# wakensky/parameter_server

Measured on AMD Instinct MI355X. Metric: aggregated kv-pairs/s (device-resident), N-way sparse push merge at 1/2/4/8 GPU, higher is better.
Workload: dtype f32; 1 GPU; cfg2: 8 pushes x 131072 sorted unique uint64 keys + f32 values, 10% shared keys (U=956,827); 64 such (channel,time) aggregates per GPU per step; global_batch=64, input_layout=arena, parallelism=key-range shards evenDivide(1); worker-sliced ingress, no data-path collective

## Files before the change

### include/psg.h

```cpp
#ifndef PSG_H_
#define PSG_H_

#include <stddef.h>
#include <stdint.h>

#ifdef __cplusplus
extern "C" {
#endif

#define PSG_ABI_VERSION 1
#define PSG_MAX_VALUE_ARRAYS 4

typedef enum psg_status {
  PSG_OK = 0,
  PSG_ERR_ARG = -1,
  PSG_ERR_UNMATCHED = -2,
  PSG_ERR_RANGE = -3,
  PSG_ERR_NO_TIME = -4,
  PSG_ERR_OOM = -5,
  PSG_ERR_DEVICE = -6,
  PSG_ERR_UNSORTED = -7,
  PSG_ERR_SIZE = -8,
  PSG_ERR_CHANNEL = -9,
  PSG_ERR_EMPTY_KEYS = -10,
// ... 77 lines not shown

int psg_plan_create(int device, int dtype, int m, unsigned flags,
                    const psg_merge_job* jobs, int njobs, psg_plan** out);
int psg_plan_max_push(void);
int psg_plan_run(psg_plan* plan, void* stream);
int psg_plan_run_stage(psg_plan* plan, int stage, void* stream);
int psg_plan_matched(psg_plan* plan, uint64_t* matched);
#define PSG_KERNEL_TILE 0
#define PSG_KERNEL_TILE64 1
#define PSG_KERNEL_PACKED 2
#define PSG_KERNEL_DENSE 3
#define PSG_KERNEL_CURSOR 4
#define PSG_KERNEL_PACKED_CURSOR 5
int psg_plan_form(psg_plan* plan, int* form);
int psg_plan_bytes(psg_plan* plan, uint64_t* bytes, uint64_t* kv_pairs);
int psg_plan_destroy(psg_plan* plan);

int psg_gather_dev(int dtype, const uint64_t* dkeys, uint64_t nd,
                   const void* dvals, const uint64_t* req, uint64_t nreq,
                   void* out, unsigned long long* matched, void* stream);

int psg_key_union_dev(const uint64_t* a, uint64_t na, const uint64_t* b,
                      uint64_t nb, uint64_t* out, uint64_t* nout,
                      void* stream);

typedef struct psg_nway psg_nway;
int psg_nway_max_push(void);
int psg_nway_create(int device, int dtype, int m, unsigned flags, int npush,
                    const uint64_t* const* keys, const uint64_t* n, const void* const* vals,
                    uint64_t* out_keys, void* const* out_vals, psg_nway** out);
// ... 188 lines not shown
```

### parameter_server_amd/_lib.py

```python
from __future__ import annotations

import ctypes as C
import os

_HERE = os.path.dirname(os.path.abspath(__file__))
LIB_PATH = os.environ.get("PSG_LIB_PATH") or os.path.join(_HERE, "libpsg.so")

PSG_OK = 0
PSG_ERR_ARG = -1
PSG_ERR_UNMATCHED = -2
PSG_ERR_RANGE = -3
PSG_ERR_NO_TIME = -4
PSG_ERR_OOM = -5
PSG_ERR_DEVICE = -6
PSG_ERR_UNSORTED = -7
PSG_ERR_SIZE = -8
PSG_ERR_CHANNEL = -9
PSG_ERR_EMPTY_KEYS = -10
PSG_ERR_SIGNATURE = -11
PSG_KC_SIG = 1
PSG_KC_KEYS = 2
PSG_KC_ERASE = 4
PSG_MAX_SIG_LEN = 2048

# ... 81 lines not shown
    "psg_key_cache_clear": (C.c_int, [_p, C.c_int]),
    "psg_push_compressed": (C.c_int, [_p, C.c_int, C.c_int, _u64, _u64, _p, _sz, C.c_int,
                                      _p, _p]),
    "psg_key_cache_bytes": (C.c_int, [_p, C.c_int, _psz]),
    "psg_received_shape": (C.c_int, [_p, C.c_int, C.POINTER(C.c_int), _psz, _psz]),
    "psg_received": (C.c_int, [_p, C.c_int, C.c_int, C.POINTER(_p)]),
    "psg_gather": (C.c_int, [_p, C.c_int, _p, _sz, _p, _psz]),
    "psg_plan_create": (C.c_int, [C.c_int, C.c_int, C.c_int, C.c_uint,
                                  C.POINTER(MergeJob), C.c_int, C.POINTER(_p)]),
    "psg_plan_max_push": (C.c_int, []),
    "psg_plan_run": (C.c_int, [_p, _p]),
    "psg_plan_run_stage": (C.c_int, [_p, C.c_int, _p]),
    "psg_plan_matched": (C.c_int, [_p, _pu64]),
    "psg_plan_bytes": (C.c_int, [_p, _pu64, _pu64]),
    "psg_plan_form": (C.c_int, [_p, C.POINTER(C.c_int)]),
    "psg_plan_destroy": (C.c_int, [_p]),
    "psg_gather_dev": (C.c_int, [C.c_int, _p, _u64, _p, _p, _u64, _p, _p, _p]),
    "psg_key_union_dev": (C.c_int, [_p, _u64, _p, _u64, _p, _pu64, _p]),
    "psg_shard_bounds": (C.c_int, [_sz, _pu64]),
    "psg_slice_dev": (C.c_int, [_p, _u64, _u64, _u64, _p, C.c_int, _p, _p]),
    "psg_crc32c_dev": (C.c_int, [_p, _p, _u64, _u64, _p, _p, _p]),
    "psg_snappy_uncompress_dev": (C.c_int, [_p, _p, _u64, _p, _p, _p, _p]),
    "psg_snappy_uncompressed_length": (C.c_int, [_p, _sz, _psz]),
    "psg_freq_resize": (C.c_int, [_p, C.c_int, C.c_int, C.c_int]),
    "psg_freq_clear": (C.c_int, [_p, C.c_int]),
    "psg_freq_empty": (C.c_int, [_p, C.c_int, C.POINTER(C.c_int)]),
    "psg_freq_insert": (C.c_int, [_p, C.c_int, _p, _p, _sz]),
    "psg_freq_query": (C.c_int, [_p, C.c_int, _p, _sz, C.c_int, _p, _psz]),
    "psg_freq_insert_dev": (C.c_int, [_p, C.c_int, _p, _p, _sz, _p]),
    "psg_freq_query_scratch_bytes": (_sz, [_sz]),
# ... 125 lines not shown
```

### parameter_server_amd/csrc/psg_device.h

```cpp
#pragma once
#include <hip/hip_runtime.h>
#include <stdint.h>

namespace psg {
namespace dev {

__device__ __forceinline__ uint64_t wave_search(const uint64_t* __restrict__ S,
                                                uint64_t n, uint64_t key,
                                                bool upper, int lane) {
  uint64_t lo = 0, hi = n;
  while (hi > lo) {
    const uint64_t len = hi - lo;
    const uint64_t step = (len + 63) >> 6;
    const uint64_t idx = lo + (uint64_t)(lane + 1) * step - 1;
    bool pred = true;
    if (idx < hi) {
      const uint64_t s = S[idx];
      pred = upper ? (s > key) : (s >= key);
    }
    const unsigned long long mask = __ballot(pred);
    if (mask == 0) {
      lo = hi;
      break;
    }
// ... 93 lines not shown
      if (lane >= d) s += y;
    }
    if (lane < kW) wsum[lane] = s;
  }
  __syncthreads();
  *total = wsum[kW - 1];
  return (w > 0 ? wsum[w - 1] : 0u) + x - v;
}

__device__ __forceinline__ uint32_t bucket_scale(uint64_t r32, uint32_t nb) {
  const float f = (float)nb * 4294967296.0f * (1.0f - 0x1p-20f) *
                  __builtin_amdgcn_rcpf((float)(r32 + 1ull));
  return f >= 4294967295.0f ? 0xffffffffu : (uint32_t)f;
}

template <typename V>
__device__ __forceinline__ V fold_step(V acc, int lp, int p, V v,
                                       bool parallel, bool cont) {
  if (p == 0 && !cont) return v;
  if (!parallel) {
    const bool gap = (lp >= 0) ? (p - lp > 1) : (cont && p > 0);
    if (gap) acc = acc + V(0);
  }
  return acc + v;
}


}
}
```

### parameter_server_amd/csrc/psg_internal.h

```cpp
#pragma once

#include <hip/hip_runtime.h>
#include <stdint.h>

namespace psg {

constexpr int kMaxPush = 4096;
constexpr int kMaxM = 4;
constexpr int kTileSlots = 1024;
#ifndef PSG_PACK_TS
#define PSG_PACK_TS 2048
#endif
constexpr int kPackTileSlots = PSG_PACK_TS;
constexpr int kWideSlots = 2048;

constexpr uint32_t kFlagParallel = 1u;
constexpr uint32_t kFlagCont = 2u;
constexpr uint32_t kFlagLastTile = 4u;

enum PartMode : uint32_t { kSearch = 0, kStream = 1 };
constexpr uint32_t kStreamChunk = 512;

struct JobDev {
  const uint64_t* dkeys;
// ... 53 lines not shown
struct DenseCheck {
  const uint64_t* keys;
  uint64_t n;
  const uint64_t* D;
  uint64_t nd;
  unsigned long long* out;
};

hipError_t launch_partition(const JobDev* d_jobs, const uint32_t* d_split_item_job,
                            uint32_t nsplit_items, const uint64_t* d_items,
                            uint32_t nitems, hipStream_t stream, bool xcd = false);
hipError_t launch_aggregate_tile(int dtype, int m, const TileDesc* d_tiles, uint32_t ntiles,
                                 int form, hipStream_t stream);
uint32_t bucket_index_words(uint32_t tile_slots);
hipError_t launch_bucket_index(const TileDesc* d_tiles, uint32_t ntiles, uint32_t tile_slots,
                               uint32_t* out,
                               hipStream_t stream);
constexpr int kPackCursorPushes = 256;
hipError_t launch_aggregate_tile_packed(int dtype, int m, const TileDesc* d_tiles,
                                        uint32_t ntiles, hipStream_t stream,
                                        const CursorChunk* d_chunks = nullptr,
                                        uint32_t nchunks = 0, uint32_t* bx = nullptr);
hipError_t launch_aggregate_dense(int dtype, int m, const TileDesc* d_tiles, uint32_t ntiles,
                                  hipStream_t stream);
hipError_t launch_dense_check(const DenseCheck* checks, uint32_t nchecks, const uint64_t* items,
                              uint64_t nitems, hipStream_t stream);
hipError_t launch_gather(int dtype, const uint64_t* dkeys, uint64_t nd,
                         const void* dvals, const uint64_t* req, uint64_t nreq,
                         void* out, unsigned long long* matched,
                         hipStream_t stream);
struct HostCopyDesc {
// ... 116 lines not shown
```

### parameter_server_amd/csrc/psg_runtime.hip

```cpp
#include <hip/hip_runtime.h>
#include <chrono>

#include <algorithm>
#include <cmath>
#include <iterator>
#include <cstdarg>
#include <cstdio>
#include <cstdlib>
#include <cstring>
#include <deque>
#include <map>
#include <memory>
#include <mutex>
#include <string>
#include <unordered_map>
#include <vector>

#include "../../include/psg.h"
#include "psg_host.h"
#include "psg_internal.h"

using psg::JobDev;

namespace {
// ... 120 lines not shown
  std::vector<JobDev> h;
  struct JobInfo {
    uint32_t np = 0, ntiles = 0;
    std::vector<uint64_t> pn;
    std::vector<uint32_t> slot;
    uint32_t ncaller = 0;
    uint32_t* seg = nullptr;
    uint32_t segq = 1;
    unsigned long long* fail = nullptr;
    uint32_t kr = 0;
    uint32_t nch = 0;
  };
  std::vector<JobInfo> info;
  uint32_t ntiles = 0, nitems = 0, nsplit = 0;
  bool split_once = false;
  bool all_search = false;
  void* blob = nullptr;
  size_t blob_bytes = 0;
  JobDev* d_jobs = nullptr;
  psg::TileDesc* d_tiles = nullptr;
  uint32_t* d_split_items = nullptr;
  uint64_t* d_items = nullptr;
  char* himg[2] = {nullptr, nullptr};
  const void* himg_dev[2] = {nullptr, nullptr};
  bool zero_copy = true;
  size_t himg_cap[2] = {0, 0};
  hipEvent_t himg_ev[2] = {nullptr, nullptr};
  int himg_cur = 0;

  std::vector<uint64_t> last_shape;
// ... 138 lines not shown
      for (JobInfo& I : info) {
        I.nch = (uint32_t)((I.ntiles + per - 1) / per);
        nc += I.nch;
      }
      nchunks = (uint32_t)nc;
    } else {
      nchunks = 0;
    }
    size_t off = align_up(sizeof(JobDev) * jobs.size(), 256);
    const size_t tiles_off = off;
    off = align_up(off + sizeof(psg::TileDesc) * tiles, 256);
    const bool use_index = index && !dense;
    const uint32_t iw = psg::bucket_index_words(tile);
    const size_t index_off = off;
    if (use_index) off = align_up(off + 4 * (size_t)iw * tiles, 256);
    const size_t sitems_off = off;
    off = align_up(off + 4 * sitems, 256);
    const size_t items_off = off;
    off = align_up(off + 8 * items, 256);
    const size_t cjobs_off = off;
    if (cursor) off = align_up(off + sizeof(psg::CursorJob) * jobs.size(), 256);
    const size_t chunks_off = off;
    if (cursor || pcursor) off = align_up(off + sizeof(psg::CursorChunk) * nchunks, 256);
    const size_t zero_off = off;
    size_t fail_cur = zero_off;
    {
      uint64_t npall = 0;
      for (const JobInfo& I : info) npall += I.np;
      off = align_up(off + 8 * npall, 256);
    }
// ... 45 lines not shown
    if (himg_ev[ib]) HIP_TRY(hipEventSynchronize(himg_ev[ib]));
    else HIP_TRY(hipEventCreateWithFlags(&himg_ev[ib], hipEventDisableTiming));
    if (off > himg_cap[ib]) {
      if (himg[ib]) HIP_TRY(hipHostFree(himg[ib]));
      himg[ib] = nullptr;
      himg_cap[ib] = 0;
      HIP_TRY(hipHostMalloc((void**)&himg[ib], off));
      himg_cap[ib] = off;
      himg_dev[ib] = nullptr;
      void* dp = nullptr;
      if (hipHostGetDevicePointer(&dp, himg[ib], 0) == hipSuccess) himg_dev[ib] = dp;
      else (void)hipGetLastError();
    }
    char* img = himg[ib];
    memset(img + zero_off, 0, zero_end - zero_off);
    psg::TileDesc* htiles = (psg::TileDesc*)(img + tiles_off);
    uint32_t* hsitems = (uint32_t*)(img + sitems_off);
    uint64_t* hitems = (uint64_t*)(img + items_off);
    uint64_t tcur = 0, icur = 0, scur = 0;
    for (size_t j = 0; j < jobs.size(); ++j) {
      const JobSpec& s = jobs[j];
      JobInfo& I = info[j];
      const Offs& o = offs[j];
      const uint32_t np = I.np, nt = I.ntiles;
      uint64_t* hk = (uint64_t*)(img + o.pk);
      uint64_t* hv = (uint64_t*)(img + o.pv);
      for (uint32_t p = 0; p < np; ++p) {
        const uint32_t c = I.slot[p];
        hk[p] = (uint64_t)s.pkeys[c];
        for (int i = 0; i < m; ++i) hv[(size_t)p * m + i] = (uint64_t)s.pvals[(size_t)c * m + i];
// ... 147 lines not shown
      cb.d[1] = psg::HostCopyDesc{(const char*)himg_dev[ib] + zero_off, base + zero_off,
                                  (uint64_t)(off - zero_off)};
      HIP_TRY(psg::launch_host_copy_batch(cb, strm));
    } else if (same) {
      HIP_TRY(hipMemcpyAsync(blob, img, tiles_off, hipMemcpyHostToDevice, strm));
      HIP_TRY(hipMemcpyAsync(base + zero_off, img + zero_off, off - zero_off,
                             hipMemcpyHostToDevice, strm));
    } else if (zc_ok) {
      HIP_TRY(psg::launch_host_copy(blob, himg_dev[ib], off, strm));
    } else {
      HIP_TRY(hipMemcpyAsync(blob, img, off, hipMemcpyHostToDevice, strm));
    }
    if (cacheable) last_shape.swap(shape);
    else last_shape.clear();
    HIP_TRY(hipEventRecord(himg_ev[ib], strm));
    if (use_index)
      HIP_TRY(psg::launch_bucket_index(d_tiles, ntiles, tile,
                                       (uint32_t*)((char*)blob + index_off), strm));
    split_once = index && nsplit > 0 && !dense && !cursor && !pcursor;
    all_search = true;
    for (const JobDev& d : h) all_search = all_search && d.mode == psg::kSearch;
    if (split_once)
      HIP_TRY(psg::launch_partition(d_jobs, d_split_items, nsplit, nullptr, 0, strm));
    if (!async) HIP_TRY(hipStreamSynchronize(strm));
    return PSG_OK;
  }

  int run_stage(int stage, hipStream_t s) const {
    if (h.empty()) return PSG_OK;
    if (stage == 0) {
      if (cursor || pcursor)
        HIP_TRY(hipMemsetAsync(d_zero, 0, zero_bytes, s));
      else if (!dense)
        HIP_TRY(psg::launch_partition(d_jobs, d_split_items, split_once ? 0u : nsplit, d_items,
                                      nitems, s, all_search));
    } else if (cursor)
      HIP_TRY(psg::launch_aggregate_cursor(dtype, m, (int)ckr, d_cjobs, d_chunks, nchunks, d_bx, s));
    else if (dense)
      HIP_TRY(psg::launch_aggregate_dense(dtype, m, d_tiles, ntiles, s));
// ... 783 lines not shown
  return PSG_OK;
}

int psg_plan_form(psg_plan* plan, int* form) {
  if (!plan || !form) return fail(PSG_ERR_ARG, "null argument");
  const JobTable& T = plan->table;
  *form = T.cursor ? PSG_KERNEL_CURSOR
          : T.pcursor ? PSG_KERNEL_PACKED_CURSOR
          : T.dense ? PSG_KERNEL_DENSE
          : T.pack  ? PSG_KERNEL_PACKED
          : T.wide  ? PSG_KERNEL_TILE64
                    : PSG_KERNEL_TILE;
  return PSG_OK;
}

int psg_plan_bytes(psg_plan* plan, uint64_t* bytes, uint64_t* kv) {
  if (!plan) return fail(PSG_ERR_ARG, "null plan");
  if (bytes) *bytes = plan->bytes;
  if (kv) *kv = plan->kv;
  return PSG_OK;
}

int psg_plan_destroy(psg_plan* plan) {
  if (!plan) return PSG_OK;
  (void)hipSetDevice(plan->table.device);
  plan->table.release();
  delete plan;
  return PSG_OK;
}

// ... 1415 lines not shown
```

### parameter_server_amd/csrc/psg_tile.hip

```cpp
#include <hip/hip_runtime.h>
#include <stdint.h>

#include "psg_device.h"
#include "psg_internal.h"

#define AS1 __attribute__((address_space(1)))
#ifndef KCAP64
#define KCAP64 7
#endif

namespace psg {

#ifndef PSG_SKELETON
#define PSG_SKELETON 0
#endif
#ifdef PSG_PHASES
constexpr int kPhTiles = 1 << 17;
__device__ uint32_t g_phase[kPhTiles][8];
#define PH(i) do { const unsigned long long _t = clock64(); \
    ph_acc[i] += (uint32_t)(_t - ph_t); ph_t = _t; } while (0)
#else
#define PH(i) do { } while (0)
#endif

// ... 144 lines not shown
                                 __HIP_MEMORY_SCOPE_AGENT);
        const uint32_t len = b > a ? (b - a < (uint32_t)kTS ? b - a : (uint32_t)kTS) : 0u;
        pln[lane] = len;
        pkp[lane] = (uint64_t)(kp + a);
#pragma unroll
        for (int mi = 0; mi < M; ++mi) pvp[lane * M + mi] = (uint64_t)(vp[mi] + a);
        nr = (len + 63u) >> 6;
      }
      const uint32_t x = wave_scan_incl(nr);
      if (lane < kGroup) rpre[lane + 1] = x;
      if (lane == 0) rpre[0] = 0;
    }
  };
  const uint32_t s0 = 4u * (uint32_t)tid;
  const uint32_t* Bg = T.bt;
  const bool dma = PSG_DDMA && nt == (uint32_t)kTS && ((uintptr_t)Dg & 15u) == 0u &&
                   ((uintptr_t)Bg & 15u) == 0u;
  auto issue_dma = [&]() {
#pragma unroll
    for (int j = 0; j < 2; ++j) {
      const uint32_t c = 2u * w + (uint32_t)j;
      dma16(Dg + 128u * c + 2u * (uint32_t)lane, (char*)dk + 1024u * c);
    }
    static_assert(kNB / 512 <= kNW, "one 1-KB unit of the bucket table per wave at most");
    if (Bg && w < (uint32_t)kNB / 512u)
      dma16((const char*)Bg + 1024u * w + 16u * (uint32_t)lane, (char*)bt32 + 1024u * w);
  };
  if (dma && w != 0) issue_dma();
  if (np) load_tables(0);
  if (dma && w == 0) issue_dma();
  if (!dma) {
    uint64_t d[4];
    if (s0 + 3u < nt && ((uintptr_t)Dg & 15u) == 0u) {
      const u64x2 x0 = __builtin_nontemporal_load((const AS1 u64x2*)(Dg + s0));
      const u64x2 x1 = __builtin_nontemporal_load((const AS1 u64x2*)(Dg + s0 + 2));
      d[0] = x0.x; d[1] = x0.y; d[2] = x1.x; d[3] = x1.y;
    } else {
#pragma unroll
      for (int j = 0; j < 4; ++j) d[j] = s0 + j < nt ? G(Dg)[s0 + j] : ~0ull;
    }
    u32x2 btw = {0u, 0u};
    if (Bg) btw = __builtin_nontemporal_load((const AS1 u32x2*)Bg + tid);
#pragma unroll
    for (int j = 0; j < 4; ++j) dk[s0 + j] = d[j];
    if (Bg) {
      bt32[tid * (kBPT / 2)] = btw.x;
      bt32[tid * (kBPT / 2) + 1] = btw.y;
    }
    __builtin_amdgcn_s_waitcnt(0x0f70);
  }
  if (cont) {
    V a0[M][4];
#pragma unroll
    for (int mi = 0; mi < M; ++mi)
#pragma unroll
      for (int j = 0; j < 4; ++j)
        a0[mi][j] = s0 + j < nt ? G((const V*)T.out[mi] + T.slot0)[s0 + j] : V(0);
    __builtin_amdgcn_s_waitcnt(0x0f70);
    if constexpr (kFuse) {
      *(u32x4*)&cnt32[8 * tid] = u32x4{__float_as_uint(a0[0][0]), 0u, __float_as_uint(a0[0][1]), 0u};
      *(u32x4*)&cnt32[8 * tid + 4] = u32x4{__float_as_uint(a0[0][2]), 0u, __float_as_uint(a0[0][3]), 0u};
    } else {
#pragma unroll
// ... 6 lines not shown
    *(u32x4*)&cnt32[8 * tid + 4] = u32x4{0u, 0u, 0u, 0u};
  } else {
#pragma unroll
    for (int mi = 0; mi < M; ++mi)
#pragma unroll
      for (int j = 0; j < 4; ++j) acc[mi][s0 + j] = V(0);
  }
  if constexpr (kFuse) {
  } else if constexpr (kCntW) {
    *(u32x4*)&cnt32[4 * tid] = u32x4{0u, 0u, 0u, 0u};
  } else {
    cnt32[2 * tid] = 0u;
    cnt32[2 * tid + 1] = 0u;
  }
  if (tid < 4) dk[kTS + tid] = ~0ull;
  if (Bg) {
    if (tid == 0) bt[kNB] = (uint16_t)nt;
  } else {
    uint32_t z = 0;
#pragma unroll
    for (int i = 0; i < kBPT / 2; ++i) bt32[tid * (kBPT / 2) + i] = z;
  }
  if (tid == 0) pcarry = -1;
  if (dma)
    lds_barrier();
  else
    __syncthreads();
  PH(0);

  uint32_t done = 0, U = np ? uni(rpre[np < (uint32_t)kGroup ? np : kGroup]) : 0u;
  uint32_t g0 = 0;
  uint32_t nrw = 0, ua = 0, Rw = 0;
  uint32_t re[kCap];
// ... 55 lines not shown
  const uint64_t klo = uni64(dk[0]);
  const uint64_t khi = uni64(dk[nt - 1]);
  const uint64_t range = khi - klo;
  const int bits = range ? 64 - __builtin_clzll(range) : 0;
  const int s2 = bits > 32 ? bits - 32 : 0;
  const uint64_t r32 = range >> s2;
  const uint32_t mul = dev::bucket_scale(r32, kNB);
  auto bucket = [&](uint64_t k) -> uint32_t {
    const uint64_t x = (k - klo) >> s2;
    const uint32_t xs = x > r32 ? 0xffffffffu : (uint32_t)x;
    const uint32_t b = __umulhi(xs, mul);
    return b < (uint32_t)(kNB - 1) ? b : (uint32_t)(kNB - 1);
  };


  if (!Bg) {
  const u64x2 y0 = *(const u64x2*)&dk[s0];
  const u64x2 y1 = *(const u64x2*)&dk[s0 + 2];
  const uint64_t dd[4] = {y0.x, y0.y, y1.x, y1.y};
#pragma unroll
  for (int j = 0; j < 4; ++j)
    if (s0 + j < nt)
    {
      const uint32_t b = bucket(dd[j]);
      __hip_atomic_fetch_add(&bt32[b >> 1], 1u << (16 * (b & 1u)), __ATOMIC_RELAXED,
                             __HIP_MEMORY_SCOPE_WORKGROUP);
    }
  __syncthreads();
  {
    uint32_t e[kBPT];
#pragma unroll
// ... 226 lines not shown
    } else {
#pragma unroll
      for (int j = 0; j < 4; ++j)
        if (s0 + j < nt) GW(o)[j] = res[mi][j];
    }
  }
  PH(6);
#ifdef PSG_PHASES
  if (tid == 0 && ti < (uint32_t)kPhTiles)
    for (int i = 0; i < 8; ++i) g_phase[ti][i] = ph_acc[i];
#endif
}

template <int kTSl>
__global__ __launch_bounds__(kTSl / 4) void bucket_index_kernel(
    const TileDesc* __restrict__ tiles, uint32_t ntiles, uint32_t* __restrict__ out) {
  constexpr int kNT = kTSl / 4;
  constexpr int kNW = kNT / 64;
  constexpr int kNB = kTSl;
  constexpr int kBPT = kNB / kNT;
  __shared__ __attribute__((aligned(16))) uint32_t bt32[(kNB + 8) / 2];
  __shared__ uint32_t wsum[kNW];
  const uint32_t ti = blockIdx.x;
  if (ti >= ntiles) return;
  const TileDesc& T = tiles[ti];
  const uint32_t nt = T.nt;
  const uint64_t* Dg = T.dk;
  const int tid = threadIdx.x, lane = tid & 63;
  const uint32_t w = uni((uint32_t)tid >> 6);
  const uint32_t s0 = 4u * (uint32_t)tid;
  const uint64_t klo = G(Dg)[0];
  const uint64_t khi = G(Dg)[nt - 1];
  const uint64_t range = khi - klo;
  const int bits = range ? 64 - __builtin_clzll(range) : 0;
  const int s2 = bits > 32 ? bits - 32 : 0;
  const uint64_t r32 = range >> s2;
  const uint32_t mul = dev::bucket_scale(r32, kNB);
#pragma unroll
  for (int i = 0; i < kBPT / 2; ++i) bt32[tid * (kBPT / 2) + i] = 0u;
  __syncthreads();
#pragma unroll
  for (int j = 0; j < 4; ++j)
    if (s0 + j < nt) {
      const uint64_t x = (G(Dg)[s0 + j] - klo) >> s2;
      const uint32_t b = x > r32 ? (uint32_t)(kNB - 1) : __umulhi((uint32_t)x, mul);
      __hip_atomic_fetch_add(&bt32[b >> 1], 1u << (16 * (b & 1u)), __ATOMIC_RELAXED,
                             __HIP_MEMORY_SCOPE_WORKGROUP);
    }
  __syncthreads();
  uint32_t e[kBPT];
#pragma unroll
  for (int i = 0; i < kBPT / 2; ++i) {
    const uint32_t h = bt32[tid * (kBPT / 2) + i];
    e[2 * i] = h & 0xffffu;
    e[2 * i + 1] = h >> 16;
  }
  uint32_t tot = 0;
#pragma unroll
  for (int j = 0; j < kBPT; ++j) {
    const uint32_t c = e[j];
    e[j] = tot;
    tot += c;
  }
  const uint32_t x = wave_scan_incl(tot);
  if (lane == 63) wsum[w] = x;
  __syncthreads();
  uint32_t off = x - tot;
#pragma unroll
  for (uint32_t v = 0; v < (uint32_t)kNW - 1u; ++v) off += v < w ? wsum[v] : 0u;
  uint32_t* o = out + (size_t)ti * (kNB / 2);
#pragma unroll
  for (int i = 0; i < kBPT / 2; ++i)
    o[tid * (kBPT / 2) + i] = (e[2 * i] + off) | (e[2 * i + 1] + off) << 16;
}

#ifndef PSG_PAD_LDS
#define PSG_PAD_LDS 0
#endif
template <typename V, int M>
hipError_t go(const TileDesc* t, uint32_t n, int form, hipStream_t s) {
  if (form == 1)
    hipLaunchKernelGGL((tile_kernel<V, M, 64>), dim3(n), dim3(nt_of(64)), PSG_PAD_LDS, s, t, n);
  else
    hipLaunchKernelGGL((tile_kernel<V, M, 32>), dim3(n), dim3(nt_of(32)), PSG_PAD_LDS, s, t, n);
  return hipGetLastError();
}

template <typename V>
// ... 4 lines not shown
    case 3: return go<V, 3>(t, n, form, s);
    case 4: return go<V, 4>(t, n, form, s);
    default: return hipErrorInvalidValue;
  }
}

}

#ifdef PSG_PHASES
extern "C" int psg_debug_phases(uint32_t* out, uint32_t ntiles) {
  if (ntiles > (uint32_t)kPhTiles) ntiles = kPhTiles;
  return hipMemcpyFromSymbol(out, HIP_SYMBOL(g_phase), (size_t)ntiles * 32) == hipSuccess ? 0 : -1;
}
#endif

uint32_t bucket_index_words(uint32_t tile_slots) { return tile_slots / 2u; }

hipError_t launch_bucket_index(const TileDesc* d_tiles, uint32_t ntiles, uint32_t tile_slots,
                               uint32_t* out, hipStream_t stream) {
  if (ntiles == 0) return hipSuccess;
  switch (tile_slots) {
    case 1024:
      hipLaunchKernelGGL(bucket_index_kernel<1024>, dim3(ntiles), dim3(256), 0, stream, d_tiles,
                         ntiles, out);
      break;
    case 2048:
      hipLaunchKernelGGL(bucket_index_kernel<2048>, dim3(ntiles), dim3(512), 0, stream, d_tiles,
                         ntiles, out);
      break;
    case 4096:
      hipLaunchKernelGGL(bucket_index_kernel<4096>, dim3(ntiles), dim3(1024), 0, stream, d_tiles,
                         ntiles, out);
      break;
    default:
      return hipErrorInvalidValue;
  }
  return hipGetLastError();
}

hipError_t launch_aggregate_tile(int dtype, int m, const TileDesc* d_tiles, uint32_t ntiles,
                                 int form, hipStream_t stream) {
  if (ntiles == 0) return hipSuccess;
  return dtype == 0 ? launch_m<float>(m, d_tiles, ntiles, form, stream)
                    : launch_m<double>(m, d_tiles, ntiles, form, stream);
}

}
// ... 1 lines not shown
```

### parameter_server_amd/csrc/psg_tile_cursor.hip

```cpp
#include <hip/hip_runtime.h>
#include <stdint.h>

#include "psg_device.h"
#include "psg_internal.h"

#define AS1 __attribute__((address_space(1)))

namespace psg {

namespace {

template <typename T>
__device__ __forceinline__ const AS1 T* G(const T* p) {
  return (const AS1 T*)p;
}
template <typename T>
__device__ __forceinline__ AS1 T* GW(T* p) {
  return (AS1 T*)p;
}

constexpr int kTS = kTileSlots;
constexpr int kNT = kTS / 4;
constexpr int kNW = kNT / 64;
constexpr int kNB = kTS;
// ... 157 lines not shown
      }
      if (g0 == 0) {
        uint64_t d[4];
        if (s0 + 3u < nt && ((uintptr_t)Dg & 15u) == 0u) {
          const u64x2 x0 = __builtin_nontemporal_load((const AS1 u64x2*)(Dg + s0));
          const u64x2 x1 = __builtin_nontemporal_load((const AS1 u64x2*)(Dg + s0 + 2));
          d[0] = x0.x; d[1] = x0.y; d[2] = x1.x; d[3] = x1.y;
        } else {
#pragma unroll
          for (int j = 0; j < 4; ++j) {
            uint64_t o = ~0ull;
            asm volatile("" : "+v"(o));
            d[j] = s0 + j < nt ? G(Dg)[s0 + j] : o;
          }
        }
        const u32x2 btw =
            __builtin_nontemporal_load((const AS1 u32x2*)(J.bt + (size_t)t * (kNB / 2)) + tid);
        V a0[M][4];
#pragma unroll
        for (int mi = 0; mi < M; ++mi)
#pragma unroll
          for (int j = 0; j < 4; ++j)
            a0[mi][j] = (cont && s0 + j < nt) ? G((const V*)J.out[mi] + slot0)[s0 + j] : V(0);
#pragma unroll
        for (int j = 0; j < 4; ++j) {
          dk[s0 + j] = d[j];
#pragma unroll
          for (int mi = 0; mi < M; ++mi) acc[mi][s0 + j] = a0[mi][j];
        }
        {
          uint32_t z = 0, o = ~0u;
          asm volatile("" : "+v"(z), "+v"(o));
          *(u32x4*)&cnt[s0] = u32x4{z, z, z, z};
          if (tid < 4) dk[kTS + tid] = (uint64_t)o << 32 | o;
        }
        *(u32x2*)&bt32[2 * tid] = btw;
        if (tid == 0) bt[kNB] = (uint16_t)nt;
        __syncthreads();
      }

      uint32_t inp = 0;
      uint32_t ends[kPPW];
      uint32_t ovf = 0;
#pragma unroll
      for (int p = 0; p < kPPW; ++p) {
        ends[p] = qc[p];
        bool closed = qn[p] >= np;
#pragma unroll
        for (int r = 0; r < kRR; ++r) {
          const int rr = p * kRR + r;
          if ((uint32_t)r < kr && !closed) {
            const bool in = ((hv >> rr) & 1u) && (open || ek[rr] < nxt);
            const uint64_t out = __ballot(!in);
// ... 228 lines not shown
```

### parameter_server_amd/csrc/psg_tile_packed.hip

```cpp
#include <hip/hip_runtime.h>
#include <stdint.h>

#include "psg_device.h"
#include "psg_internal.h"

#define AS1 __attribute__((address_space(1)))

namespace psg {

namespace {

template <typename T>
__device__ __forceinline__ const AS1 T* G(const T* p) {
  return (const AS1 T*)p;
}
template <typename T>
__device__ __forceinline__ AS1 T* GW(T* p) {
  return (AS1 T*)p;
}

#ifndef PSG_SKELETON
#define PSG_SKELETON 0
#endif

// ... 330 lines not shown
      emax = y > emax ? y : emax;
    }
    if (in) {
      pre[ql + 1] = X;
#pragma nounroll
      for (uint32_t e = X - lv; e < X; ++e) ep[e] = (uint8_t)ql;
    }
    if (lane_id() == 0u) {
      __hip_atomic_fetch_add(&gsh[0], fit, __ATOMIC_RELAXED, __HIP_MEMORY_SCOPE_WORKGROUP);
      __hip_atomic_fetch_max(&gsh[1], emax, __ATOMIC_RELAXED, __HIP_MEMORY_SCOPE_WORKGROUP);
    }
    if (t == 0u) pre[0] = 0;
  };
  const uint32_t s0i = 4u * (uint32_t)tid;
  const uint32_t* Bg = T.bt;
  const bool dma = !CUR && PSG_DDMA && nt == (uint32_t)kTS && ((uintptr_t)Dg & 15u) == 0u &&
                   ((uintptr_t)Bg & 15u) == 0u;
  auto issue_dma = [&]() {
#pragma unroll
    for (int j = 0; j < 2; ++j) {
      const uint32_t c = 2u * w + (uint32_t)j;
      dma16(Dg + 128u * c + 2u * (uint32_t)lane, (char*)dk + 1024u * c);
    }
    static_assert(kNB / 512 <= kNW, "one 1-KB unit of the bucket table per wave at most");
    if (Bg && w < (uint32_t)kNB / 512u)
      dma16((const char*)Bg + 1024u * w + 16u * (uint32_t)lane, (char*)bt32 + 1024u * w);
  };
  if (dma && w >= 2) issue_dma();
  if (np) {
    if constexpr (!CUR) tables_a(0);
  }
  if (dma && w < 2) issue_dma();
  if (!dma) {
    uint64_t d[4];
    if (s0i + 3u < nt && ((uintptr_t)Dg & 15u) == 0u) {
      const u64x2 x0 = *(const AS1 u64x2*)(Dg + s0i);
      const u64x2 x1 = *(const AS1 u64x2*)(Dg + s0i + 2);
      d[0] = x0.x; d[1] = x0.y; d[2] = x1.x; d[3] = x1.y;
    } else {
#pragma unroll
      for (int j = 0; j < 4; ++j) d[j] = s0i + j < nt ? G(Dg)[s0i + j] : ~0ull;
    }
    u32x2 btw = {0u, 0u};
    if (Bg) btw = __builtin_nontemporal_load((const AS1 u32x2*)Bg + tid);
#pragma unroll
    for (int j = 0; j < 4; ++j) dk[s0i + j] = d[j];
    if (Bg) *(u32x2*)&bt[tid * kBPT] = btw;
    __builtin_amdgcn_s_waitcnt(0x0f70);
  }
  uint32_t cx = 0, clv = 0;
  if constexpr (CUR) {
    if (np) clv = cur_a(0, true, &cx);
  }

  uint32_t ones = ~0u, one = 1u;
  if constexpr (CUR) asm volatile("" : "+v"(ones), "+v"(one));
  if (cont) {
    V a0[M][4];
#pragma unroll
    for (int mi = 0; mi < M; ++mi)
#pragma unroll
      for (int j = 0; j < 4; ++j)
// ... 4 lines not shown
#pragma unroll
      for (int j = 0; j < 4; ++j) acc[mi][s0i + j] = a0[mi][j];
  } else {
#pragma unroll
    for (int mi = 0; mi < M; ++mi)
#pragma unroll
      for (int j = 0; j < 4; ++j) acc[mi][s0i + j] = V(0);
  }
#pragma unroll
  for (int j = 0; j < 4; ++j) lastl[s0i + j] = (uint16_t)one;
  if (tid < 8) dk[kTS + tid] = (uint64_t)ones << 32 | ones;
  {
    uint32_t z = 0;
    asm volatile("" : "+v"(z));
    if (!Bg) *(u32x2*)&bt[tid * kBPT] = u32x2{z, z};
    if (Bg && tid == 0) bt[kNB] = (uint16_t)nt;
  }
  if (tid == 0) pcarry = (int)ones;
  if (dma)
    lds_barrier();
  else
    __syncthreads();
  if (np) {
    if constexpr (CUR) cur_b(0, clv, cx);
    else tables_b(0);
  }
  if (dma)
    lds_barrier();
  else
    __syncthreads();

// ... 92 lines not shown
        e[j] = tot;
        tot += c;
      }
      const uint32_t x = wave_scan_incl(tot);
      if (lane_id() == 63u) wsum[w] = x;
      __syncthreads();
      uint32_t off = x - tot;
#pragma unroll
      for (uint32_t v = 0; v < (uint32_t)kNW - 1u; ++v) off += v < w ? wsum[v] : 0u;
      const u32x2 o = {(e[0] + off) | (e[1] + off) << 16, (e[2] + off) | (e[3] + off) << 16};
      *(u32x2*)&bt[t * kBPT] = o;
      if (t == 0) bt[kNB] = (uint16_t)nt;
    }
    __syncthreads();
  };
  if (!Bg) build_bt(false);

  for (;;) {
    if (!U) {
      g0 += gp;
      if (g0 >= np) break;
#pragma unroll
      for (int j = 0; j < 4; ++j) lastl[s0i + j] = lastl[s0i + j] == gp + 1u ? 1 : 0;
      if constexpr (CUR) {
        uint32_t x;
        const uint32_t lv = cur_a(g0, false, &x);
        __syncthreads();
        cur_b(g0, lv, x);
      } else {
        tables_a(g0);
        __syncthreads();
// ... 167 lines not shown
                  if (j < lane && s == sl) lowest = false;
                }
                if (lowest) {
                  apply();
                  pend = false;
                }
              }
            }
          }
        }
        if (w == wl && lane == 63) pcarry = mylast;
      }
      __syncthreads();
    }
    if (done + kNW * Rw < U || g0 + gp < np) {
      if (Bg) {
        const uint32_t t = 64u * w + lane_id();
        *(u32x2*)&bt[t * kBPT] = __builtin_nontemporal_load((const AS1 u32x2*)Bg + t);
        __syncthreads();
      } else {
        build_bt(true);
      }
    }

    done += kNW * Rw;
    if (done < U) {
      load_pass();
      continue;
    }
    U = 0;
    if (w == 0 && lane_id() == 0u) pcarry = -1;
  }

// ... 96 lines not shown
```

### parameter_server_amd/kv_vector.py

```python
from __future__ import annotations

import ctypes as C
from dataclasses import dataclass, field
from typing import List, Optional, Sequence

import numpy as np

from . import _lib
from ._lib import PSG_F32, PSG_F64, PSG_PARALLEL_MATCH, PSG_SERIAL_MATCH

KEY_ALL = (0, (1 << 64) - 1)


def _np_dtype(dtype: int):
    return np.float32 if dtype == PSG_F32 else np.float64


def _ptr(a: np.ndarray) -> int:
    return a.ctypes.data


@dataclass
class Message:

# ... 165 lines not shown
            cj[j].push_n = C.cast(pn, C.POINTER(C.c_uint64))
            cj[j].out = C.cast(out, C.POINTER(C.c_void_p))
        h = C.c_void_p()
        flags = (flags & ~PSG_PARALLEL_MATCH) | (PSG_PARALLEL_MATCH if parallel_match
                                                 else PSG_SERIAL_MATCH)
        _lib.check(self._L.psg_plan_create(device, dtype, m, flags, cj, len(jobs),
                                           C.byref(h)))
        self._h = h
        self.npush_total = sum(len(J["push_keys"]) for J in jobs)
        b, kv = C.c_uint64(), C.c_uint64()
        _lib.check(self._L.psg_plan_bytes(h, C.byref(b), C.byref(kv)))
        self.bytes, self.kv_pairs = b.value, kv.value
        f = C.c_int()
        _lib.check(self._L.psg_plan_form(h, C.byref(f)))
        self.form = f.value

    def run(self, stream: Optional[int] = None) -> None:
        _lib.check(self._L.psg_plan_run(self._h, stream or None))

    def run_stage(self, stage: int, stream: Optional[int] = None) -> None:
        _lib.check(self._L.psg_plan_run_stage(self._h, stage, stream or None))

    def matched(self) -> np.ndarray:
        out = np.zeros(max(1, self.npush_total), np.uint64)
        _lib.check(self._L.psg_plan_matched(
            self._h, out.ctypes.data_as(C.POINTER(C.c_uint64))))
        return out[: self.npush_total]

    def close(self):
        if getattr(self, "_h", None):
# ... 103 lines not shown
```

Measured before the change: 182.6 billion kv-pairs/s.

## Compress bucket index to 4-bit counts decoded in-kernel with wave scan

```diff
diff --git a/include/psg.h b/include/psg.h
--- a/include/psg.h
+++ b/include/psg.h
@@ -115,6 +115,7 @@
 #define PSG_KERNEL_PACKED_CURSOR 5
 int psg_plan_form(psg_plan* plan, int* form);
 int psg_plan_bytes(psg_plan* plan, uint64_t* bytes, uint64_t* kv_pairs);
+int psg_plan_index_info(psg_plan* plan, uint64_t* index_bytes, uint64_t* marked_tiles);
 int psg_plan_destroy(psg_plan* plan);
 
 int psg_gather_dev(int dtype, const uint64_t* dkeys, uint64_t nd,
diff --git a/parameter_server_amd/_lib.py b/parameter_server_amd/_lib.py
--- a/parameter_server_amd/_lib.py
+++ b/parameter_server_amd/_lib.py
@@ -119,6 +119,7 @@
     "psg_plan_matched": (C.c_int, [_p, _pu64]),
     "psg_plan_bytes": (C.c_int, [_p, _pu64, _pu64]),
     "psg_plan_form": (C.c_int, [_p, C.POINTER(C.c_int)]),
+    "psg_plan_index_info": (C.c_int, [_p, _pu64, _pu64]),
     "psg_plan_destroy": (C.c_int, [_p]),
     "psg_gather_dev": (C.c_int, [C.c_int, _p, _u64, _p, _p, _u64, _p, _p, _p]),
     "psg_key_union_dev": (C.c_int, [_p, _u64, _p, _u64, _p, _pu64, _p]),
diff --git a/parameter_server_amd/csrc/psg_device.h b/parameter_server_amd/csrc/psg_device.h
--- a/parameter_server_amd/csrc/psg_device.h
+++ b/parameter_server_amd/csrc/psg_device.h
@@ -131,6 +131,78 @@
   return f >= 4294967295.0f ? 0xffffffffu : (uint32_t)f;
 }
 
+template <int kNB>
+struct BucketIndexWords {
+  static_assert(kNB == 1024 || kNB == 2048 || kNB == 4096, "8, 16 or 32 B per lane");
+  uint32_t x[kNB / 512];
+};
+
+template <int kNB>
+__device__ __forceinline__ BucketIndexWords<kNB> bucket_index_load(const uint32_t* ix, int lane) {
+  typedef uint32_t v2 __attribute__((ext_vector_type(2)));
+  typedef uint32_t v4 __attribute__((ext_vector_type(4)));
+  BucketIndexWords<kNB> r;
+  if constexpr (kNB == 1024) {
+    const v2 a = __builtin_nontemporal_load(
+        (const __attribute__((address_space(1))) v2*)ix + lane);
+    r.x[0] = a.x; r.x[1] = a.y;
+  } else {
+#pragma unroll
+    for (int i = 0; i < kNB / 2048; ++i) {
+      const v4 a = __builtin_nontemporal_load(
+          (const __attribute__((address_space(1))) v4*)ix + lane * (kNB / 2048) + i);
+      r.x[4 * i] = a.x; r.x[4 * i + 1] = a.y; r.x[4 * i + 2] = a.z; r.x[4 * i + 3] = a.w;
+    }
+  }
+  return r;
+}
+
+__device__ __forceinline__ uint32_t wave_scan_incl_dpp(uint32_t x) {
+  x += (uint32_t)__builtin_amdgcn_update_dpp(0, (int)x, 0x111, 0xf, 0xf, false);
+  x += (uint32_t)__builtin_amdgcn_update_dpp(0, (int)x, 0x112, 0xf, 0xf, false);
+  x += (uint32_t)__builtin_amdgcn_update_dpp(0, (int)x, 0x114, 0xf, 0xf, false);
+  x += (uint32_t)__builtin_amdgcn_update_dpp(0, (int)x, 0x118, 0xf, 0xf, false);
+  x += (uint32_t)__builtin_amdgcn_update_dpp(0, (int)x, 0x142, 0xa, 0xf, false);
+  x += (uint32_t)__builtin_amdgcn_update_dpp(0, (int)x, 0x143, 0xc, 0xf, false);
+  return x;
+}
+
+template <int kNB>
+__device__ __forceinline__ void bucket_index_decode(const BucketIndexWords<kNB>& ix,
+                                                    uint32_t* bt32, uint32_t nt, int lane) {
+  typedef uint32_t v4 __attribute__((ext_vector_type(4)));
+  constexpr int W = kNB / 512;
+  const bool marked = ((uint32_t)__builtin_amdgcn_readfirstlane((int)ix.x[0]) & 15u) == 15u;
+  uint32_t ev[W], od[W], before[W], tot = 0;
+#pragma unroll
+  for (int i = 0; i < W; ++i) {
+    const uint32_t lo = ix.x[i] & 0x0f0f0f0fu, hi = (ix.x[i] >> 4) & 0x0f0f0f0fu;
+    const uint32_t s = (lo + hi) * 0x01010101u;
+    ev[i] = s - lo - hi;
+    od[i] = s - hi;
+    before[i] = tot;
+    tot += s >> 24;
+  }
+  const uint32_t off = wave_scan_incl_dpp(tot) - tot;
+#pragma unroll
+  for (int i = 0; i < W; ++i) {
+    const uint32_t base = (off + before[i]) * 0x00010001u;
+    v4 o;
+    o.x = ((ev[i] & 0xffu) | (od[i] & 0xffu) << 16) + base;
+    o.y = ((ev[i] >> 8 & 0xffu) | (od[i] >> 8 & 0xffu) << 16) + base;
+    o.z = ((ev[i] >> 16 & 0xffu) | (od[i] >> 16 & 0xffu) << 16) + base;
+    o.w = ((ev[i] >> 24) | (od[i] >> 24) << 16) + base;
+    if (marked) o = v4{0u, 0u, 0u, 0u};
+    *(v4*)&bt32[4 * (lane * W + i)] = o;
+  }
+  if (lane == 0) bt32[kNB / 2] = nt | (marked ? 0x10000u : 0u);
+}
+
+template <int kNB>
+__device__ __forceinline__ bool bucket_index_marked(const uint32_t* bt32) {
+  return ((uint32_t)__builtin_amdgcn_readfirstlane((int)bt32[kNB / 2]) >> 16) != 0u;
+}
+
 template <typename V>
 __device__ __forceinline__ V fold_step(V acc, int lp, int p, V v,
                                        bool parallel, bool cont) {
diff --git a/parameter_server_amd/csrc/psg_internal.h b/parameter_server_amd/csrc/psg_internal.h
--- a/parameter_server_amd/csrc/psg_internal.h
+++ b/parameter_server_amd/csrc/psg_internal.h
@@ -91,7 +91,7 @@
                                  int form, hipStream_t stream);
 uint32_t bucket_index_words(uint32_t tile_slots);
 hipError_t launch_bucket_index(const TileDesc* d_tiles, uint32_t ntiles, uint32_t tile_slots,
-                               uint32_t* out,
+                               uint32_t* out, unsigned long long* nmarked,
                                hipStream_t stream);
 constexpr int kPackCursorPushes = 256;
 hipError_t launch_aggregate_tile_packed(int dtype, int m, const TileDesc* d_tiles,
diff --git a/parameter_server_amd/csrc/psg_runtime.hip b/parameter_server_amd/csrc/psg_runtime.hip
--- a/parameter_server_amd/csrc/psg_runtime.hip
+++ b/parameter_server_amd/csrc/psg_runtime.hip
@@ -158,6 +158,7 @@
   std::vector<JobInfo> info;
   uint32_t ntiles = 0, nitems = 0, nsplit = 0;
   bool split_once = false;
+  uint64_t index_bytes = 0, marked_tiles = 0;
   bool all_search = false;
   void* blob = nullptr;
   size_t blob_bytes = 0;
@@ -326,6 +327,8 @@
     const uint32_t iw = psg::bucket_index_words(tile);
     const size_t index_off = off;
     if (use_index) off = align_up(off + 4 * (size_t)iw * tiles, 256);
+    const size_t marked_off = off;
+    if (use_index) off += 256;
     const size_t sitems_off = off;
     off = align_up(off + 4 * sitems, 256);
     const size_t items_off = off;
@@ -401,6 +404,7 @@
     }
     char* img = himg[ib];
     memset(img + zero_off, 0, zero_end - zero_off);
+    if (use_index) memset(img + marked_off, 0, 8);
     psg::TileDesc* htiles = (psg::TileDesc*)(img + tiles_off);
     uint32_t* hsitems = (uint32_t*)(img + sitems_off);
     uint64_t* hitems = (uint64_t*)(img + items_off);
@@ -578,15 +582,26 @@
     if (cacheable) last_shape.swap(shape);
     else last_shape.clear();
     HIP_TRY(hipEventRecord(himg_ev[ib], strm));
+    index_bytes = 0;
+    marked_tiles = 0;
     if (use_index)
       HIP_TRY(psg::launch_bucket_index(d_tiles, ntiles, tile,
-                                       (uint32_t*)((char*)blob + index_off), strm));
+                                       (uint32_t*)((char*)blob + index_off),
+                                       (unsigned long long*)((char*)blob + marked_off), strm));
     split_once = index && nsplit > 0 && !dense && !cursor && !pcursor;
     all_search = true;
     for (const JobDev& d : h) all_search = all_search && d.mode == psg::kSearch;
     if (split_once)
       HIP_TRY(psg::launch_partition(d_jobs, d_split_items, nsplit, nullptr, 0, strm));
     if (!async) HIP_TRY(hipStreamSynchronize(strm));
+    if (use_index) {
+      index_bytes = 4 * (uint64_t)iw * tiles;
+      if (tiles) {
+        HIP_TRY(hipMemcpyAsync(&marked_tiles, (char*)blob + marked_off, 8, hipMemcpyDeviceToHost,
+                               strm));
+        HIP_TRY(hipStreamSynchronize(strm));
+      }
+    }
     return PSG_OK;
   }
 
@@ -1400,6 +1415,13 @@
   return PSG_OK;
 }
 
+int psg_plan_index_info(psg_plan* plan, uint64_t* index_bytes, uint64_t* marked_tiles) {
+  if (!plan) return fail(PSG_ERR_ARG, "null plan");
+  if (index_bytes) *index_bytes = plan->table.index_bytes;
+  if (marked_tiles) *marked_tiles = plan->table.marked_tiles;
+  return PSG_OK;
+}
+
 int psg_plan_bytes(psg_plan* plan, uint64_t* bytes, uint64_t* kv) {
   if (!plan) return fail(PSG_ERR_ARG, "null plan");
   if (bytes) *bytes = plan->bytes;
diff --git a/parameter_server_amd/csrc/psg_tile.hip b/parameter_server_amd/csrc/psg_tile.hip
--- a/parameter_server_amd/csrc/psg_tile.hip
+++ b/parameter_server_amd/csrc/psg_tile.hip
@@ -182,21 +182,24 @@
   };
   const uint32_t s0 = 4u * (uint32_t)tid;
   const uint32_t* Bg = T.bt;
-  const bool dma = PSG_DDMA && nt == (uint32_t)kTS && ((uintptr_t)Dg & 15u) == 0u &&
-                   ((uintptr_t)Bg & 15u) == 0u;
+  const bool dma = PSG_DDMA && nt == (uint32_t)kTS && ((uintptr_t)Dg & 15u) == 0u;
   auto issue_dma = [&]() {
 #pragma unroll
     for (int j = 0; j < 2; ++j) {
       const uint32_t c = 2u * w + (uint32_t)j;
       dma16(Dg + 128u * c + 2u * (uint32_t)lane, (char*)dk + 1024u * c);
     }
-    static_assert(kNB / 512 <= kNW, "one 1-KB unit of the bucket table per wave at most");
-    if (Bg && w < (uint32_t)kNB / 512u)
-      dma16((const char*)Bg + 1024u * w + 16u * (uint32_t)lane, (char*)bt32 + 1024u * w);
   };
-  if (dma && w != 0) issue_dma();
-  if (np) load_tables(0);
-  if (dma && w == 0) issue_dma();
+  constexpr uint32_t kIxWave = (uint32_t)kNW - 1u;
+  if (dma && w != 0 && w != kIxWave) issue_dma();
+  if (w == kIxWave) {
+    if (Bg) dev::bucket_index_decode<kNB>(dev::bucket_index_load<kNB>(Bg, lane), bt32, nt, lane);
+    if (dma) issue_dma();
+  }
+  if (w == 0) {
+    if (np) load_tables(0);
+    if (dma) issue_dma();
+  }
   if (!dma) {
     uint64_t d[4];
     if (s0 + 3u < nt && ((uintptr_t)Dg & 15u) == 0u) {
@@ -207,14 +210,8 @@
 #pragma unroll
       for (int j = 0; j < 4; ++j) d[j] = s0 + j < nt ? G(Dg)[s0 + j] : ~0ull;
     }
-    u32x2 btw = {0u, 0u};
-    if (Bg) btw = __builtin_nontemporal_load((const AS1 u32x2*)Bg + tid);
 #pragma unroll
     for (int j = 0; j < 4; ++j) dk[s0 + j] = d[j];
-    if (Bg) {
-      bt32[tid * (kBPT / 2)] = btw.x;
-      bt32[tid * (kBPT / 2) + 1] = btw.y;
-    }
     __builtin_amdgcn_s_waitcnt(0x0f70);
   }
   if (cont) {
@@ -251,9 +248,7 @@
     cnt32[2 * tid + 1] = 0u;
   }
   if (tid < 4) dk[kTS + tid] = ~0ull;
-  if (Bg) {
-    if (tid == 0) bt[kNB] = (uint16_t)nt;
-  } else {
+  if (!Bg) {
     uint32_t z = 0;
 #pragma unroll
     for (int i = 0; i < kBPT / 2; ++i) bt32[tid * (kBPT / 2) + i] = z;
@@ -339,7 +334,7 @@
   };
 
 
-  if (!Bg) {
+  if (!Bg || dev::bucket_index_marked<kNB>(bt32)) {
   const u64x2 y0 = *(const u64x2*)&dk[s0];
   const u64x2 y1 = *(const u64x2*)&dk[s0 + 2];
   const uint64_t dd[4] = {y0.x, y0.y, y1.x, y1.y};
@@ -596,20 +591,18 @@
 
 template <int kTSl>
 __global__ __launch_bounds__(kTSl / 4) void bucket_index_kernel(
-    const TileDesc* __restrict__ tiles, uint32_t ntiles, uint32_t* __restrict__ out) {
+    const TileDesc* __restrict__ tiles, uint32_t ntiles, uint32_t* __restrict__ out,
+    unsigned long long* __restrict__ nmarked) {
   constexpr int kNT = kTSl / 4;
-  constexpr int kNW = kNT / 64;
   constexpr int kNB = kTSl;
   constexpr int kBPT = kNB / kNT;
   __shared__ __attribute__((aligned(16))) uint32_t bt32[(kNB + 8) / 2];
-  __shared__ uint32_t wsum[kNW];
   const uint32_t ti = blockIdx.x;
   if (ti >= ntiles) return;
   const TileDesc& T = tiles[ti];
   const uint32_t nt = T.nt;
   const uint64_t* Dg = T.dk;
-  const int tid = threadIdx.x, lane = tid & 63;
-  const uint32_t w = uni((uint32_t)tid >> 6);
+  const int tid = threadIdx.x;
   const uint32_t s0 = 4u * (uint32_t)tid;
   const uint64_t klo = G(Dg)[0];
   const uint64_t khi = G(Dg)[nt - 1];
@@ -630,30 +623,21 @@
                              __HIP_MEMORY_SCOPE_WORKGROUP);
     }
   __syncthreads();
-  uint32_t e[kBPT];
+  static_assert(kBPT == 4, "one u16 of nibbles per thread");
+  uint32_t nib = 0;
+  bool big = false;
 #pragma unroll
   for (int i = 0; i < kBPT / 2; ++i) {
     const uint32_t h = bt32[tid * (kBPT / 2) + i];
-    e[2 * i] = h & 0xffffu;
-    e[2 * i + 1] = h >> 16;
-  }
-  uint32_t tot = 0;
-#pragma unroll
-  for (int j = 0; j < kBPT; ++j) {
-    const uint32_t c = e[j];
-    e[j] = tot;
-    tot += c;
-  }
-  const uint32_t x = wave_scan_incl(tot);
-  if (lane == 63) wsum[w] = x;
-  __syncthreads();
-  uint32_t off = x - tot;
-#pragma unroll
-  for (uint32_t v = 0; v < (uint32_t)kNW - 1u; ++v) off += v < w ? wsum[v] : 0u;
-  uint32_t* o = out + (size_t)ti * (kNB / 2);
-#pragma unroll
-  for (int i = 0; i < kBPT / 2; ++i)
-    o[tid * (kBPT / 2) + i] = (e[2 * i] + off) | (e[2 * i + 1] + off) << 16;
+    const uint32_t c0 = h & 0xffffu, c1 = h >> 16;
+    big |= c0 > 14u || c1 > 14u;
+    nib |= ((c0 < 14u ? c0 : 14u) | (c1 < 14u ? c1 : 14u) << 4) << (8 * i);
+  }
+  const bool marked = __syncthreads_or(big) != 0;
+  if (marked && tid < 2) nib = 0xffffu;
+  ((uint16_t*)(out + (size_t)ti * (kNB / 8)))[tid] = (uint16_t)nib;
+  if (marked && tid == 0)
+    __hip_atomic_fetch_add(GW(nmarked), 1ull, __ATOMIC_RELAXED, __HIP_MEMORY_SCOPE_AGENT);
 }
 
 #ifndef PSG_PAD_LDS
@@ -688,23 +672,24 @@
 }
 #endif
 
-uint32_t bucket_index_words(uint32_t tile_slots) { return tile_slots / 2u; }
+uint32_t bucket_index_words(uint32_t tile_slots) { return tile_slots / 8u; }
 
 hipError_t launch_bucket_index(const TileDesc* d_tiles, uint32_t ntiles, uint32_t tile_slots,
-                               uint32_t* out, hipStream_t stream) {
+                               uint32_t* out, unsigned long long* nmarked,
+                               hipStream_t stream) {
   if (ntiles == 0) return hipSuccess;
   switch (tile_slots) {
     case 1024:
       hipLaunchKernelGGL(bucket_index_kernel<1024>, dim3(ntiles), dim3(256), 0, stream, d_tiles,
-                         ntiles, out);
+                         ntiles, out, nmarked);
       break;
     case 2048:
       hipLaunchKernelGGL(bucket_index_kernel<2048>, dim3(ntiles), dim3(512), 0, stream, d_tiles,
-                         ntiles, out);
+                         ntiles, out, nmarked);
       break;
     case 4096:
       hipLaunchKernelGGL(bucket_index_kernel<4096>, dim3(ntiles), dim3(1024), 0, stream, d_tiles,
-                         ntiles, out);
+                         ntiles, out, nmarked);
       break;
     default:
       return hipErrorInvalidValue;
diff --git a/parameter_server_amd/csrc/psg_tile_cursor.hip b/parameter_server_amd/csrc/psg_tile_cursor.hip
--- a/parameter_server_amd/csrc/psg_tile_cursor.hip
+++ b/parameter_server_amd/csrc/psg_tile_cursor.hip
@@ -195,8 +195,8 @@
             d[j] = s0 + j < nt ? G(Dg)[s0 + j] : o;
           }
         }
-        const u32x2 btw =
-            __builtin_nontemporal_load((const AS1 u32x2*)(J.bt + (size_t)t * (kNB / 2)) + tid);
+        dev::BucketIndexWords<kNB> ix;
+        if (w == 0) ix = dev::bucket_index_load<kNB>(J.bt + (size_t)t * (kNB / 8), lane);
         V a0[M][4];
 #pragma unroll
         for (int mi = 0; mi < M; ++mi)
@@ -215,9 +215,39 @@
           *(u32x4*)&cnt[s0] = u32x4{z, z, z, z};
           if (tid < 4) dk[kTS + tid] = (uint64_t)o << 32 | o;
         }
-        *(u32x2*)&bt32[2 * tid] = btw;
-        if (tid == 0) bt[kNB] = (uint16_t)nt;
+        if (w == 0) dev::bucket_index_decode<kNB>(ix, bt32, nt, lane);
         __syncthreads();
+        if (dev::bucket_index_marked<kNB>(bt32)) {
+#pragma unroll
+          for (int j = 0; j < 4; ++j)
+            if (s0 + j < nt) {
+              const uint32_t b = bucket(dk[s0 + j]);
+              __hip_atomic_fetch_add(&bt32[b >> 1], 1u << (16 * (b & 1u)), __ATOMIC_RELAXED,
+                                     __HIP_MEMORY_SCOPE_WORKGROUP);
+            }
+          __syncthreads();
+          const u32x2 h = *(const u32x2*)&bt32[2 * tid];
+          uint32_t e[4] = {h.x & 0xffffu, h.x >> 16, h.y & 0xffffu, h.y >> 16};
+          uint32_t tot = 0;
+#pragma unroll
+          for (int j = 0; j < 4; ++j) {
+            const uint32_t c = e[j];
+            e[j] = tot;
+            tot += c;
+          }
+          uint32_t* const wsum = cnt;
+          const uint32_t x = dev::wave_scan_incl_dpp(tot);
+          if (lane == 63) wsum[w] = x;
+          __syncthreads();
+          uint32_t off = x - tot;
+#pragma unroll
+          for (uint32_t v = 0; v < (uint32_t)kNW - 1u; ++v) off += v < w ? wsum[v] : 0u;
+          __syncthreads();
+          if (tid < kNW) wsum[tid] = 0u;
+          *(u32x2*)&bt32[2 * tid] =
+              u32x2{(e[0] + off) | (e[1] + off) << 16, (e[2] + off) | (e[3] + off) << 16};
+          __syncthreads();
+        }
       }
 
       uint32_t inp = 0;
diff --git a/parameter_server_amd/csrc/psg_tile_packed.hip b/parameter_server_amd/csrc/psg_tile_packed.hip
--- a/parameter_server_amd/csrc/psg_tile_packed.hip
+++ b/parameter_server_amd/csrc/psg_tile_packed.hip
@@ -368,19 +368,19 @@
   };
   const uint32_t s0i = 4u * (uint32_t)tid;
   const uint32_t* Bg = T.bt;
-  const bool dma = !CUR && PSG_DDMA && nt == (uint32_t)kTS && ((uintptr_t)Dg & 15u) == 0u &&
-                   ((uintptr_t)Bg & 15u) == 0u;
+  const bool dma = !CUR && PSG_DDMA && nt == (uint32_t)kTS && ((uintptr_t)Dg & 15u) == 0u;
   auto issue_dma = [&]() {
 #pragma unroll
     for (int j = 0; j < 2; ++j) {
       const uint32_t c = 2u * w + (uint32_t)j;
       dma16(Dg + 128u * c + 2u * (uint32_t)lane, (char*)dk + 1024u * c);
     }
-    static_assert(kNB / 512 <= kNW, "one 1-KB unit of the bucket table per wave at most");
-    if (Bg && w < (uint32_t)kNB / 512u)
-      dma16((const char*)Bg + 1024u * w + 16u * (uint32_t)lane, (char*)bt32 + 1024u * w);
   };
-  if (dma && w >= 2) issue_dma();
+  if (dma && w > 2) issue_dma();
+  if (w == 2) {
+    if (Bg) dev::bucket_index_decode<kNB>(dev::bucket_index_load<kNB>(Bg, lane), bt32, nt, lane);
+    if (dma) issue_dma();
+  }
   if (np) {
     if constexpr (!CUR) tables_a(0);
   }
@@ -395,11 +395,8 @@
 #pragma unroll
       for (int j = 0; j < 4; ++j) d[j] = s0i + j < nt ? G(Dg)[s0i + j] : ~0ull;
     }
-    u32x2 btw = {0u, 0u};
-    if (Bg) btw = __builtin_nontemporal_load((const AS1 u32x2*)Bg + tid);
 #pragma unroll
     for (int j = 0; j < 4; ++j) dk[s0i + j] = d[j];
-    if (Bg) *(u32x2*)&bt[tid * kBPT] = btw;
     __builtin_amdgcn_s_waitcnt(0x0f70);
   }
   uint32_t cx = 0, clv = 0;
@@ -434,7 +431,6 @@
     uint32_t z = 0;
     asm volatile("" : "+v"(z));
     if (!Bg) *(u32x2*)&bt[tid * kBPT] = u32x2{z, z};
-    if (Bg && tid == 0) bt[kNB] = (uint16_t)nt;
   }
   if (tid == 0) pcarry = (int)ones;
   if (dma)
@@ -557,7 +553,7 @@
     }
     __syncthreads();
   };
-  if (!Bg) build_bt(false);
+  if (!Bg || dev::bucket_index_marked<kNB>(bt32)) build_bt(false);
 
   for (;;) {
     if (!U) {
@@ -755,9 +751,11 @@
       __syncthreads();
     }
     if (done + kNW * Rw < U || g0 + gp < np) {
-      if (Bg) {
-        const uint32_t t = 64u * w + lane_id();
-        *(u32x2*)&bt[t * kBPT] = __builtin_nontemporal_load((const AS1 u32x2*)Bg + t);
+      if (Bg && !dev::bucket_index_marked<kNB>(bt32)) {
+        if (w == 2) {
+          const int l = (int)lane_id();
+          dev::bucket_index_decode<kNB>(dev::bucket_index_load<kNB>(Bg, l), bt32, nt, l);
+        }
         __syncthreads();
       } else {
         build_bt(true);
diff --git a/parameter_server_amd/kv_vector.py b/parameter_server_amd/kv_vector.py
--- a/parameter_server_amd/kv_vector.py
+++ b/parameter_server_amd/kv_vector.py
@@ -203,6 +203,9 @@
         f = C.c_int()
         _lib.check(self._L.psg_plan_form(h, C.byref(f)))
         self.form = f.value
+        ib, mt = C.c_uint64(), C.c_uint64()
+        _lib.check(self._L.psg_plan_index_info(h, C.byref(ib), C.byref(mt)))
+        self.index_bytes, self.marked_tiles = ib.value, mt.value
 
     def run(self, stream: Optional[int] = None) -> None:
         _lib.check(self._L.psg_plan_run(self._h, stream or None))
```

Measured after the change: 185.8 billion kv-pairs/s (median of 6 runs). +1.7%, better.
